# graph-embedding/node2vec

Hardware: AMD Instinct MI355X
Metric: walk-steps/sec + embedding-updates/sec on 100M-node synthetic; 1/2/4/8 GPU (higher is better)
Workload: dtype f64

## Files before the change

### node2vec_amd/csrc/n2v_walk_uniform.hip

```cpp
#include "n2v_common.h"

namespace n2v {

__device__ __forceinline__ void rank_row(const n2v_graph &g, const uint32_t *first, const uint32_t *off,
                                         uint32_t x, int64_t &vb, int &n) {
  if (x < (uint32_t)g.rank_head_n) {
    const uint64_t e = g.rank_head[x];
    vb = (int64_t)(e & N2V_HOP_ROW_MASK);
    n = (int)(e >> N2V_HOP_DEG_SHIFT);
    return;
  }
  int c = 0;
  for (int half = g.rank_classes >> 1; half > 0; half >>= 1)
    if (first[c + half] <= x) c += half;
  const uint32_t f0 = first[c], o0 = off[c];
  const uint32_t d = (off[c + 1] - o0) / (first[c + 1] - f0);
  n = (int)d;
  vb = (int64_t)(o0 + (x - f0) * d);
}

template <int kHops, int kThreads>
__global__ __launch_bounds__(kThreads, 8) void walk_uniform_kernel(
    n2v_graph g, const int32_t *__restrict__ start_ids, int64_t n_start, int32_t num_walks,
    int32_t walk_length, uint64_t seed, int32_t *__restrict__ walks_out,
    uint8_t *__restrict__ valid_out, uint32_t *__restrict__ status) {
  const int lane = threadIdx.x & 63;
  const int64_t total = n_start * (int64_t)num_walks;
  const int L1 = walk_length + 1;
  const bool base_aligned = (reinterpret_cast<uintptr_t>(walks_out) & 63u) == 0;
  extern __shared__ uint32_t rank_lds[];
  const uint32_t *cls_first = rank_lds;
  const uint32_t *cls_where = rank_lds + (kHops >= 3 ? g.rank_classes : 0);
  if (kHops >= 3) {
    for (int c = threadIdx.x; c < g.rank_classes; c += kThreads) {
      rank_lds[c] = g.rank_class_first[c];
      rank_lds[g.rank_classes + c] = g.rank_class_off[c];
    }
    __syncthreads();
  }
  const bool emit_rank = kHops == 3 && g.rank_emit != 0;
  for (;;) {
    uint32_t t = 0;
    if (lane == 0) t = atomicAdd(&status[1], 64u);
    const int64_t base = (int64_t)(uint32_t)__builtin_amdgcn_readfirstlane((int)t);
    if (base >= total) break;
    const int64_t r = base + lane;
    const bool have = r < total;
    int32_t v = -1;
    uint64_t h0 = 0;
    bool alive = have;
    if (have) {
      v = start_ids[r / num_walks];
      const int32_t ordinal = (int32_t)(r % num_walks) + 1;
      h0 = walker_stream(seed, (uint64_t)v * (uint64_t)num_walks + (uint64_t)(ordinal - 1));
      if (v < 0 || (int64_t)v >= g.n_vertices) {
        atomicOr(status, N2V_ST_RANGE);
        alive = false;
      }
    }
    int64_t vb = 0;
    int n = 0;
    int32_t v_emit = v;
    if (kHops >= 3) {
      if (alive) {
        const int32_t rk = g.rank_of[v];
        if (emit_rank) v_emit = rk;
        rank_row(g, cls_first, cls_where, (uint32_t)rk, vb, n);
        alive = n > 0;
      }
    } else if (alive) {
      vb = g.rowptr[v];
      n = (int)(g.rowptr[v + 1] - vb);
      alive = n > 0;
      if (kHops == 2 && g.hop8_rowptr) vb = g.hop8_rowptr[v];
    }
    bool walking = alive;
    const int64_t w0 = r * (int64_t)L1;
    int32_t buf[16];
#pragma unroll
    for (int k = 0; k < 16; ++k) buf[k] = -1;
    int lo = (int)(w0 & 15);
    auto put = [&](int64_t a, int32_t x) {
      const int k = (int)(a & 15);
#pragma unroll
      for (int kk = 0; kk < 16; ++kk) buf[kk] = (k == kk) ? x : buf[kk];
    };
    auto flush = [&](int64_t a) {
      const int k = (int)(a & 15);
      int32_t *sec = walks_out + (a & ~(int64_t)15);
#if defined(N2V_ABLATE_UNIFORM) && N2V_ABLATE_UNIFORM == 1
      if (buf[k] == 0x7fffffff) sec[k] = 0;
#else
      if (lo == 0 && k == 15 && base_aligned) {
#pragma unroll
        for (int u = 0; u < 4; ++u)
          reinterpret_cast<int4 *>(sec)[u] =
              make_int4(buf[4 * u], buf[4 * u + 1], buf[4 * u + 2], buf[4 * u + 3]);
      } else {
#pragma unroll
        for (int kk = 0; kk < 16; ++kk)
          if (kk >= lo && kk <= k) sec[kk] = buf[kk];
      }
#endif
      lo = 0;
    };
    if (have) {
      put(w0, alive ? v_emit : -1);
      if ((w0 & 15) == 15 || walk_length == 0) flush(w0);
    }
    for (int step = 0; step < walk_length; ++step) {
      if (ballot64(have) == 0ull) break;
      int32_t x = -1;
      if (walking) {
        const uint64_t bits = step_bits(h0, (uint32_t)step);
        const int pick = pick_index((uint32_t)(bits >> 32), n);
        if (kHops == 4) {
          const uint64_t e = reinterpret_cast<const uint64_t *>(g.rank_hops)[vb + pick];
          x = (int32_t)(uint32_t)e;
          if (step + 1 < walk_length) rank_row(g, cls_first, cls_where, (uint32_t)(e >> 32), vb, n);
        } else if (kHops == 3) {
#if defined(N2V_ABLATE_UNIFORM) && N2V_ABLATE_UNIFORM == 2
          const uint32_t xr = (uint32_t)((bits >> 7) % (uint64_t)g.n_vertices);
#else
          const uint32_t xr = g.rank_hops[vb + pick];
#endif
          x = emit_rank ? (int32_t)xr : g.rank_vertex[xr];
          if (step + 1 < walk_length) rank_row(g, cls_first, cls_where, xr, vb, n);
        } else if (kHops == 2) {
          const uint64_t h = g.hops8[vb + pick];
          const int cb = g.hop8_col_bits, rb = g.hop8_row_bits;
          x = (int32_t)(h & ((1ull << cb) - 1ull));
          vb = (int64_t)(((h >> cb) & ((1ull << rb) - 1ull)) << g.hop8_align_shift);
          const uint64_t code = h >> (cb + rb), esc = (1ull << (64 - cb - rb)) - 1ull;
          n = (int)code;
          if (code == esc) n = (int)(g.rowptr[x + 1] - g.rowptr[x]);
        } else if (kHops == 1) {
          const n2v_hop h = load_hop(g.hops + vb + pick);
          x = h.col;
          vb = hop_row(h);
          n = hop_deg(h);
        } else {
          x = g.col[vb + pick];
          if (step + 1 < walk_length) {
            vb = g.rowptr[x];
            n = (int)(g.rowptr[x + 1] - vb);
          }
        }
        if (step + 1 < walk_length && n == 0) {
          walking = false;
          alive = false;
        }
      }
      if (have) {
        const int64_t a = w0 + step + 1;
        put(a, x);
        if ((a & 15) == 15 || step + 1 == walk_length) flush(a);
      }
    }
    if (have) valid_out[r] = alive ? 1 : 0;
  }
}

}

extern "C" int n2v_walk_uniform_try(const n2v_graph *g, const int32_t *start_ids, int64_t n_start,
                                    int32_t num_walks, int32_t walk_length, double p, double q,
                                    uint64_t seed, int32_t *walks_out, uint8_t *valid_out,
                                    uint32_t *status, void *stream) {
  if (g->w != nullptr || g->w64 != nullptr || p != 1.0 || q != 1.0) return 0;
  const int64_t total = n_start * (int64_t)num_walks;
  if (total >= 0xffffff00ll) return 0;
  if (total == 0) return 1;
  const int form = g->rank_hops ? (g->rank_emit == 2 ? 4 : 3) : g->hops8 ? 2 : (g->hops ? 1 : 0);
  if (form >= 3) {
    const int P = g->rank_classes;
    if (P < 2 || P > 8192 || (P & (P - 1)) || !g->rank_of || !g->rank_class_first || !g->rank_class_off ||
        g->n_edges >= (1ll << 32) ||
        g->rank_head_n < 0 || g->rank_head_n > (1 << 22) || (g->rank_head_n > 0 && !g->rank_head) ||
        (g->rank_emit == 0 && !g->rank_vertex) || g->rank_emit < 0 || g->rank_emit > 2)
      return N2V_EINVAL;
  }
  if (form == 2 && (g->hop8_col_bits < 1 || g->hop8_row_bits < 1 ||
                    g->hop8_col_bits + g->hop8_row_bits > 62 || g->hop8_align_shift < 0 ||
                    g->hop8_align_shift > 6 || (g->hop8_align_shift > 0 && !g->hop8_rowptr)))
    return N2V_EINVAL;
  if (hipMemsetAsync(status + 1, 0, sizeof(uint32_t), (hipStream_t)stream) != hipSuccess)
    return N2V_ELAUNCH;
  int64_t blocks = (total + 255) / 256;
  if (form >= 3) {
    const size_t lds = (size_t)g->rank_classes * 8;
    const void *fn3 = form == 4 ? (const void *)n2v::walk_uniform_kernel<4, 1024>
                                : (const void *)n2v::walk_uniform_kernel<3, 1024>;
    blocks = (total + 1023) / 1024;
    const int64_t cap3 = n2v::resident_blocks(fn3, 1024, lds);
    if (blocks > cap3) blocks = cap3;
#define N2V_RANKED_LAUNCH(F)                                                                          \
  hipLaunchKernelGGL((n2v::walk_uniform_kernel<F, 1024>), dim3((unsigned)blocks), dim3(1024), lds,    \
                     (hipStream_t)stream, *g, start_ids, n_start, num_walks, walk_length, seed,       \
                     walks_out, valid_out, status)
    if (form == 4)
      N2V_RANKED_LAUNCH(4);
    else
      N2V_RANKED_LAUNCH(3);
#undef N2V_RANKED_LAUNCH
    if (hipGetLastError() != hipSuccess) return N2V_ELAUNCH;
    return 1;
  }
  const void *fn = form == 2   ? (const void *)n2v::walk_uniform_kernel<2, 256>
                   : form == 1 ? (const void *)n2v::walk_uniform_kernel<1, 256>
                               : (const void *)n2v::walk_uniform_kernel<0, 256>;
  const int64_t cap = n2v::resident_blocks(fn, 256, 0);
  if (blocks > cap) blocks = cap;
#define N2V_UNIFORM_LAUNCH(F)                                                                     \
  hipLaunchKernelGGL((n2v::walk_uniform_kernel<F, 256>), dim3((unsigned)blocks), dim3(256), 0,   \
                     (hipStream_t)stream, *g, start_ids, n_start, num_walks, walk_length, seed,  \
                     walks_out, valid_out, status)
  if (form == 2)
    N2V_UNIFORM_LAUNCH(2);
  else if (form == 1)
    N2V_UNIFORM_LAUNCH(1);
  else
    N2V_UNIFORM_LAUNCH(0);
#undef N2V_UNIFORM_LAUNCH
  if (hipGetLastError() != hipSuccess) return N2V_ELAUNCH;
  return 1;
}
```

Baseline: 46.03 billion.

## Regroup walk-path sector flushes across lanes via bpermute for coalesced stores

Moves the per-lane 16-entry path buffer into a shared helper and, by default, regroups flushes across the wavefront. Lanes that are ready to flush are enumerated with a ballot, and ds_bpermute hands each sector to four cooperating lanes, each of which writes one 16-byte quarter. Vector stores are now allowed whenever the output is 16-byte aligned and a quarter is fully covered. The goal is to turn scattered per-lane 64-byte writes into contiguous wavefront stores, paid for with extra ballots, a serial ffs loop and sixteen bpermutes per flush round. It also adds a random-hop ablation path for the kHops==4 form.

```diff
diff --git a/node2vec_amd/csrc/n2v_path_store.h b/node2vec_amd/csrc/n2v_path_store.h
--- /dev/null
+++ b/node2vec_amd/csrc/n2v_path_store.h
@@ -0,0 +1,96 @@
+#pragma once
+#include "n2v_common.h"
+
+#ifndef N2V_PATH_STORE_REGROUP
+#define N2V_PATH_STORE_REGROUP 1
+#endif
+
+namespace n2v {
+
+struct path_sector {
+  int32_t buf[16];
+
+  __device__ __forceinline__ void clear() {
+#pragma unroll
+    for (int k = 0; k < 16; ++k) buf[k] = -1;
+  }
+  __device__ __forceinline__ void put(int64_t a, int32_t x) {
+    const int k = (int)(a & 15);
+#pragma unroll
+    for (int kk = 0; kk < 16; ++kk) buf[kk] = (k == kk) ? x : buf[kk];
+  }
+};
+
+__device__ __forceinline__ void path_store_quarter(int32_t *p, int f, int lo, int k, bool vec_ok, int32_t v0,
+                                                   int32_t v1, int32_t v2, int32_t v3) {
+  if (f >= lo && f + 3 <= k && vec_ok) {
+    *reinterpret_cast<int4 *>(p) = make_int4(v0, v1, v2, v3);
+  } else {
+    if (f >= lo && f <= k) p[0] = v0;
+    if (f + 1 >= lo && f + 1 <= k) p[1] = v1;
+    if (f + 2 >= lo && f + 2 <= k) p[2] = v2;
+    if (f + 3 >= lo && f + 3 <= k) p[3] = v3;
+  }
+}
+
+__device__ __forceinline__ void path_flush(const path_sector &s, bool done, int64_t w0, int pos, int L1,
+                                           int32_t *__restrict__ walks_out, bool vec_ok) {
+#if defined(N2V_ABLATE_UNIFORM) && N2V_ABLATE_UNIFORM == 1
+  if (done) {
+    const int64_t a = w0 + pos;
+    const int k = (int)(a & 15);
+    int32_t *sec = walks_out + (a & ~(int64_t)15);
+    int32_t x = 0;
+#pragma unroll
+    for (int kk = 0; kk < 16; ++kk) x = (k == kk) ? s.buf[kk] : x;
+    if (x == 0x7fffffff) sec[k] = 0;
+  }
+#elif N2V_PATH_STORE_REGROUP == 0
+  if (done) {
+    const int64_t a = w0 + pos;
+    const int64_t sec = a & ~(int64_t)15;
+    const int k = (int)(a & 15);
+    const int lo = w0 > sec ? (int)(w0 & 15) : 0;
+#pragma unroll
+    for (int u = 0; u < 4; ++u)
+      path_store_quarter(walks_out + sec + 4 * u, 4 * u, lo, k, vec_ok, s.buf[4 * u], s.buf[4 * u + 1],
+                         s.buf[4 * u + 2], s.buf[4 * u + 3]);
+  }
+#else
+  uint64_t m = ballot64(done);
+  const int lane = lane_id();
+  const int q = lane & 3, j = lane >> 2;
+  while (m != 0ull) {
+    int o = -1;
+#pragma unroll 1
+    for (int i = 0; i < 16 && m != 0ull; ++i) {
+      const int b = __ffsll((unsigned long long)m) - 1;
+      m &= m - 1ull;
+      if (i == j) o = b;
+    }
+    const int src = (o < 0 ? lane : o) << 2;
+    int32_t v0 = 0, v1 = 0, v2 = 0, v3 = 0;
+#pragma unroll
+    for (int u = 0; u < 4; ++u) {
+      const int32_t t0 = __builtin_amdgcn_ds_bpermute(src, s.buf[4 * u]);
+      const int32_t t1 = __builtin_amdgcn_ds_bpermute(src, s.buf[4 * u + 1]);
+      const int32_t t2 = __builtin_amdgcn_ds_bpermute(src, s.buf[4 * u + 2]);
+      const int32_t t3 = __builtin_amdgcn_ds_bpermute(src, s.buf[4 * u + 3]);
+      v0 = (q == u) ? t0 : v0;
+      v1 = (q == u) ? t1 : v1;
+      v2 = (q == u) ? t2 : v2;
+      v3 = (q == u) ? t3 : v3;
+    }
+    if (o >= 0) {
+      const int64_t w0o = w0 + (int64_t)(o - lane) * (int64_t)L1;
+      const int64_t a = w0o + pos;
+      const int64_t sec = a & ~(int64_t)15;
+      const int k = (int)(a & 15);
+      const int lo = w0o > sec ? (int)(w0o & 15) : 0;
+      path_store_quarter(walks_out + sec + 4 * q, 4 * q, lo, k, vec_ok, v0, v1, v2, v3);
+    }
+  }
+#endif
+}
+
+}
diff --git a/node2vec_amd/csrc/n2v_walk_uniform.hip b/node2vec_amd/csrc/n2v_walk_uniform.hip
--- a/node2vec_amd/csrc/n2v_walk_uniform.hip
+++ b/node2vec_amd/csrc/n2v_walk_uniform.hip
@@ -1,4 +1,5 @@
 #include "n2v_common.h"
+#include "n2v_path_store.h"
 
 namespace n2v {
 
@@ -27,7 +28,7 @@
   const int lane = threadIdx.x & 63;
   const int64_t total = n_start * (int64_t)num_walks;
   const int L1 = walk_length + 1;
-  const bool base_aligned = (reinterpret_cast<uintptr_t>(walks_out) & 63u) == 0;
+  const bool vec_ok = (reinterpret_cast<uintptr_t>(walks_out) & 15u) == 0;
   extern __shared__ uint32_t rank_lds[];
   const uint32_t *cls_first = rank_lds;
   const uint32_t *cls_where = rank_lds + (kHops >= 3 ? g.rank_classes : 0);
@@ -76,38 +77,10 @@
     }
     bool walking = alive;
     const int64_t w0 = r * (int64_t)L1;
-    int32_t buf[16];
-#pragma unroll
-    for (int k = 0; k < 16; ++k) buf[k] = -1;
-    int lo = (int)(w0 & 15);
-    auto put = [&](int64_t a, int32_t x) {
-      const int k = (int)(a & 15);
-#pragma unroll
-      for (int kk = 0; kk < 16; ++kk) buf[kk] = (k == kk) ? x : buf[kk];
-    };
-    auto flush = [&](int64_t a) {
-      const int k = (int)(a & 15);
-      int32_t *sec = walks_out + (a & ~(int64_t)15);
-#if defined(N2V_ABLATE_UNIFORM) && N2V_ABLATE_UNIFORM == 1
-      if (buf[k] == 0x7fffffff) sec[k] = 0;
-#else
-      if (lo == 0 && k == 15 && base_aligned) {
-#pragma unroll
-        for (int u = 0; u < 4; ++u)
-          reinterpret_cast<int4 *>(sec)[u] =
-              make_int4(buf[4 * u], buf[4 * u + 1], buf[4 * u + 2], buf[4 * u + 3]);
-      } else {
-#pragma unroll
-        for (int kk = 0; kk < 16; ++kk)
-          if (kk >= lo && kk <= k) sec[kk] = buf[kk];
-      }
-#endif
-      lo = 0;
-    };
-    if (have) {
-      put(w0, alive ? v_emit : -1);
-      if ((w0 & 15) == 15 || walk_length == 0) flush(w0);
-    }
+    path_sector sector;
+    sector.clear();
+    if (have) sector.put(w0, alive ? v_emit : -1);
+    path_flush(sector, have && ((w0 & 15) == 15 || walk_length == 0), w0, 0, L1, walks_out, vec_ok);
     for (int step = 0; step < walk_length; ++step) {
       if (ballot64(have) == 0ull) break;
       int32_t x = -1;
@@ -115,7 +88,11 @@
         const uint64_t bits = step_bits(h0, (uint32_t)step);
         const int pick = pick_index((uint32_t)(bits >> 32), n);
         if (kHops == 4) {
+#if defined(N2V_ABLATE_UNIFORM) && N2V_ABLATE_UNIFORM == 2
+          const uint64_t e = ((bits >> 7) % (uint64_t)g.n_vertices) * 0x100000001ull;
+#else
           const uint64_t e = reinterpret_cast<const uint64_t *>(g.rank_hops)[vb + pick];
+#endif
           x = (int32_t)(uint32_t)e;
           if (step + 1 < walk_length) rank_row(g, cls_first, cls_where, (uint32_t)(e >> 32), vb, n);
         } else if (kHops == 3) {
@@ -151,11 +128,9 @@
           alive = false;
         }
       }
-      if (have) {
-        const int64_t a = w0 + step + 1;
-        put(a, x);
-        if ((a & 15) == 15 || step + 1 == walk_length) flush(a);
-      }
+      const int64_t a = w0 + step + 1;
+      if (have) sector.put(a, x);
+      path_flush(sector, have && ((a & 15) == 15 || step + 1 == walk_length), w0, step + 1, L1, walks_out, vec_ok);
     }
     if (have) valid_out[r] = alive ? 1 : 0;
   }
```

New measurement: 42.46 billion. -7.8%, worse.
